# xingchensong/TouchNet

Hardware: AMD Instinct MI355X
Metric: audio+text tokens/sec/node (packed seq, full train step) + step MFU (higher is better)
Workload: dtype bf16

## Files before the change

touchnet_amd/csrc/attn_bwd_fused.hip:

```cpp
#include "attn_common.h"

namespace tn {

namespace fusedkv {

#define TN_FKV_BLOCKS(M)                                                                                              \
  if constexpr (BLK == 0) { M("a0","a1","a2","a3","a4","a5","a6","a7","a8","a9","a10","a11","a12","a13","a14","a15"); } \
  if constexpr (BLK == 1) { M("a16","a17","a18","a19","a20","a21","a22","a23","a24","a25","a26","a27","a28","a29","a30","a31"); } \
  if constexpr (BLK == 2) { M("a32","a33","a34","a35","a36","a37","a38","a39","a40","a41","a42","a43","a44","a45","a46","a47"); } \
  if constexpr (BLK == 3) { M("a48","a49","a50","a51","a52","a53","a54","a55","a56","a57","a58","a59","a60","a61","a62","a63"); } \
  if constexpr (BLK == 4) { M("a64","a65","a66","a67","a68","a69","a70","a71","a72","a73","a74","a75","a76","a77","a78","a79"); } \
  if constexpr (BLK == 5) { M("a80","a81","a82","a83","a84","a85","a86","a87","a88","a89","a90","a91","a92","a93","a94","a95"); } \
  if constexpr (BLK == 6) { M("a96","a97","a98","a99","a100","a101","a102","a103","a104","a105","a106","a107","a108","a109","a110","a111"); } \
  if constexpr (BLK == 7) { M("a112","a113","a114","a115","a116","a117","a118","a119","a120","a121","a122","a123","a124","a125","a126","a127"); }

template <int BLK, bool FIRST>
__device__ __forceinline__ void acc_mfma(bf16x8_t a, bf16x8_t b) {
#define TN_M(...)                                                                                                     \
  if constexpr (FIRST)                                                                                                \
    asm volatile("s_nop 1\n\tv_mfma_f32_32x32x16_bf16 a[%c2:%c3], %0, %1, a[%c2:%c3]" ::"v"(a), "v"(b),             \
                 "n"(16 * BLK), "n"(16 * BLK + 15) : __VA_ARGS__);                                                    \
  else                                                                                                                \
    asm volatile("v_mfma_f32_32x32x16_bf16 a[%c2:%c3], %0, %1, a[%c2:%c3]" ::"v"(a), "v"(b), "n"(16 * BLK),          \
                 "n"(16 * BLK + 15) : __VA_ARGS__)
// ... 21 lines not shown
}

template <int K>
__device__ __forceinline__ void mfma_first(f32x16_t& d, u32x4_t a, bf16x8_t b) {
  asm volatile("s_waitcnt lgkmcnt(%3)\n\tv_mfma_f32_32x32x16_bf16 %0, %1, %2, 0" : "=&v"(d) : "v"(a), "v"(b), "n"(K));
}
template <int K>
__device__ __forceinline__ void mfma_acc(f32x16_t& d, u32x4_t a, bf16x8_t b) {
  asm volatile("s_waitcnt lgkmcnt(%3)\n\tv_mfma_f32_32x32x16_bf16 %0, %1, %2, %0" : "+v"(d) : "v"(a), "v"(b), "n"(K));
}
__device__ __forceinline__ void mfma_result_pad(f32x16_t& d) { asm volatile("s_nop 7\n\ts_nop 4" : "+v"(d)); }

constexpr int g2_ops(int g, bool mask) { return g < 4 ? 4 : g < 6 ? 3 + (mask ? 1 : 0) : 1 + (mask ? 1 : 0); }
constexpr int g2_wait(int s, bool mask) {
  int y = 0;
  if (s < 4) {
    y = 3 - s;
    for (int g = 0; g < s; ++g) y += g2_ops(g, mask);
  } else {
    y = g2_ops(s - 4, mask) - 1;
    for (int g = s - 3; g < s; ++g) y += g2_ops(g, mask);
  }
  return y;
}
static_assert(g2_wait(0, false) == 3 && g2_wait(3, false) == 12 && g2_wait(4, false) == 15 && g2_wait(7, false) == 10 &&
              g2_wait(5, true) == 15 && g2_wait(6, true) == 15 && g2_wait(7, true) == 13, "LDS wait table");

struct QStage {
  int qsb, meta, base, srow;
};

}

template <int D>
__global__ __launch_bounds__(256, 1) void attn_bwd_kv_fused_kernel(
    const bf16_t* __restrict__ Q, const bf16_t* __restrict__ K, const bf16_t* __restrict__ V,
    const bf16_t* __restrict__ dO, const float* __restrict__ LSE2, const float* __restrict__ Delta,
    bf16_t* __restrict__ dK, bf16_t* __restrict__ dV, const int* __restrict__ doc, AttnMeta meta, QView qv, int T,
    int Nh, int Nkv, float scale, float scale_log2, const bf16_t* __restrict__ rcos, const bf16_t* __restrict__ rsin) {
  using namespace fusedkv;
  static_assert(D == 128, "the fused dK/dV pass is built for head_dim 128");
  constexpr int BNK = 128, BQ = 32, NST = 4, SPT = kTile / BQ;
  constexpr int KSTEPS = D / 16, DBLK = D / 32;
  using Tile = PTile<BQ, D>;
  constexpr int IMGB = Tile::SIZE * 2;
  constexpr int NPC = Tile::NP * (BQ / 16);
  constexpr int PPW = NPC / 4;
  constexpr int IPS = 2 * PPW + 1;
  constexpr int STAGEB = 2 * IMGB + 4 * 256;
  constexpr int LCAP = 256;
  using KTile = PTile<32, D>;
  constexpr int KIMGB = KTile::SIZE * 2;
  static_assert(4 * 2 * KIMGB <= NST * STAGEB && 4 * 2 * WholeRows<D>::BYTES <= NST * STAGEB, "private images live in the ring area");
  __shared__ __attribute__((aligned(1024))) char smem[NST * STAGEB + (LCAP + NST + 1) * 16 + 16 + kListPre * 16];
  i32x4_t* slist = reinterpret_cast<i32x4_t*>(smem + NST * STAGEB);
  int* wcount = reinterpret_cast<int*>(smem + NST * STAGEB + (LCAP + NST + 1) * 16);
  i32x4_t* qent = reinterpret_cast<i32x4_t*>(smem + NST * STAGEB + (LCAP + NST + 1) * 16 + 16);

  const int tid = threadIdx.x, lane = tid & 63;
  const int wave = __builtin_amdgcn_readfirstlane(tid >> 6);
  const int l31 = lane & 31, hi = lane >> 5;
  const int kt = blockIdx.y, hk = blockIdx.x, b = blockIdx.z;
  const int G = Nh / Nkv;
  const int k0 = kt * BNK;
  const int wk0 = k0 + 32 * wave;
  const int kvrow = wk0 + l31;
  const bool kvalid = kvrow < T;

  const bool plain = qv.nseg == 1 && qv.off[0] == 0 && qv.row0[0] == 0 && qv.rows[0] == T && qv.rpb == T;
  i32x4_t ql_head = {kListPre + 1, 0, 0, 0}, ql_mine = {0, 0, 0, 0};
  if (plain) {
    const i32x4_t* ql = reinterpret_cast<const i32x4_t*>(meta.qlist) + ((size_t)b * meta.nq128 + kt) * (1 + kListPre);
    ql_head = ql[0];
    if (tid < kListPre) ql_mine = ql[1 + tid];
  }
  i32x4_t ws4[4];
#pragma unroll
  for (int w = 0; w < 4; ++w) {
    ws4[w] = i32x4_t{0x7fffffff, 0, 1, 0};
    if (k0 + 32 * w < T) ws4[w] = reinterpret_cast<const i32x4_t*>(meta.qstat)[(size_t)b * meta.nq32 + (k0 + 32 * w) / 32];
  }
  const int dkdoc = kvalid ? doc[(size_t)b * T + kvrow] : 0;
  {
    const size_t krow_elems = (size_t)Nkv * D;
    const uint32_t k_bytes = (uint32_t)min((size_t)T * krow_elems * 2, (size_t)0x7fffffff);
    const __amdgpu_buffer_rsrc_t rk =
        __builtin_amdgcn_make_buffer_rsrc((void*)(K + (size_t)b * T * krow_elems), 0, k_bytes, 0x00020000);
    const __amdgpu_buffer_rsrc_t rv =
        __builtin_amdgcn_make_buffer_rsrc((void*)(V + (size_t)b * T * krow_elems), 0, k_bytes, 0x00020000);
    const int rrk = lane >> 2;
    const uint32_t voffk = (uint32_t)(((size_t)rrk * krow_elems + 8 * ((lane & 3) ^ ((rrk >> 2) & 3))) * 2);
    char* kpriv = smem + wave * (2 * KIMGB);
#pragma unroll
    for (int pc = 0; pc < KTile::NP * 2; ++pc) {
      const int panel = pc % KTile::NP, rh = pc / KTile::NP;
      const uint32_t vo = (wk0 + 16 * rh + rrk < T) ? voffk : 0x80000000u;
      const uint32_t so = (uint32_t)((((size_t)wk0 + 16 * rh) * krow_elems + (size_t)hk * D + 32 * panel) * 2);
      char* dst = kpriv + panel * (KTile::PSTRIDE * 2) + rh * 1024;
      __builtin_amdgcn_raw_ptr_buffer_load_lds(rk, (lds_ptr_t)dst, 16, vo, so, 0, 0);
      __builtin_amdgcn_raw_ptr_buffer_load_lds(rv, (lds_ptr_t)(dst + KIMGB), 16, vo, so, 0, 0);
    }
  }
  wait_vmcnt<0>();
  asm volatile("" ::"v"(dkdoc));
  bf16x8_t kreg[KSTEPS], vreg[KSTEPS];
  {
    const PRowReader<32, D> krd(l31, hi);
    const bf16_t* ki = reinterpret_cast<const bf16_t*>(smem + wave * (2 * KIMGB));
#pragma unroll
    for (int s2 = 0; s2 < KSTEPS; ++s2) {
      kreg[s2] = krd.operand(ki, 0, s2);
      vreg[s2] = krd.operand(ki + KTile::SIZE, 0, s2);
    }
#pragma unroll
    for (int s2 = 0; s2 < KSTEPS; ++s2) asm volatile("s_waitcnt lgkmcnt(0)" : "+v"(kreg[s2]), "+v"(vreg[s2]));
  }
  const int n_pre = __builtin_amdgcn_readfirstlane(ql_head.x);
  const bool pre = n_pre <= kListPre;
  if (pre && tid < n_pre) qent[tid] = ql_mine;
  __syncthreads();

  const int* m_min = meta.tmin + (size_t)b * meta.nt;
  const int* m_max = meta.tmax + (size_t)b * meta.nt;
  const int* m_minpos = meta.tminpos + (size_t)b * meta.nt;
  const int qt_lo = k0 / kTile;
  const int t0 = 2 * kt, t1 = min(2 * kt + 1, meta.nt - 1);
  int bminpos = 0, bmax = 0, qt_end = 0;
  if (!pre) {
    bminpos = min(m_minpos[t0], m_minpos[t1]);
    bmax = max(m_max[t0], m_max[t1]);
    const int qhi64 = max(meta.kv_hi[(size_t)b * meta.nt + t0], meta.kv_hi[(size_t)b * meta.nt + t1]);
    qt_end = min(qhi64 + 1, meta.nt);
  }
  const int4 wsc = scalarize(ws4[0]);
  const int4 wsc1 = scalarize(ws4[1]), wsc2 = scalarize(ws4[2]), wsc3 = scalarize(ws4[3]);
  const int4 wsw[4] = {wsc, wsc1, wsc2, wsc3};
  int seg_lo[2], seg_n[2];
// ... 84 lines not shown
  auto issue = [&](const QStage& d, int sbase) {
    char* st = smem + sbase;
    const int left = d.meta & 0xff;
#pragma unroll
    for (int i = 0; i < PPW; ++i) {
      const int pc = wave + 4 * i, panel = pc % Tile::NP, rh = pc / Tile::NP;
      const uint32_t vo = (16 * rh + rr < left) ? voff : OOB;
      const uint32_t so = (uint32_t)d.base + (uint32_t)((16 * rh * qrow_elems + 32 * panel) * 2);
      char* dst = st + panel * (Tile::PSTRIDE * 2) + rh * 1024;
      __builtin_amdgcn_raw_ptr_buffer_load_lds(rq, (lds_ptr_t)dst, 16, vo, so, 0, 0);
      __builtin_amdgcn_raw_ptr_buffer_load_lds(rdo, (lds_ptr_t)(dst + IMGB), 16, vo, so, 0, 0);
    }
    const uint32_t va = lane < left ? (uint32_t)lane * 4 : OOB;
    __builtin_amdgcn_raw_ptr_buffer_load_lds(raux, (lds_ptr_t)(st + 2 * IMGB + 256 * wave), 4, va,
                                             wave < 2 ? (uint32_t)d.srow : (uint32_t)d.qsb * 4, 0, 0);
  };

  static_for<2 * DBLK>([&](auto I) { acc_zero<decltype(I)::value>(); });

  const PRowReader<BQ, D> rrd(l31, hi);
  const PTrReader<BQ, D> trd(lane);
  const uint32_t lds0 = (uint32_t)(size_t)(lds_ptr_t)smem;
  const uint32_t trb0 = lds0 + 2 * (uint32_t)trd.t[0], trb1 = lds0 + 2 * (uint32_t)trd.t[1];
  const uint32_t rwb0 = lds0 + 2 * (uint32_t)rrd.a[0], rwb1 = lds0 + 2 * (uint32_t)rrd.a[1];
  const uint32_t auxb = lds0 + 16 * (uint32_t)hi;

  bf16x8_t Pc[2];
  float pf[16];
  f32x16_t dPc;
  bool act_c = false;

  auto trip = [&](auto cur_t, auto next_t, auto mask_t, int qsb_n, const QStage& ahead, int sb_c, int sb_n,
                  int sb_a) {
    constexpr bool CUR = decltype(cur_t)::value, NEXT = decltype(next_t)::value, MASK = decltype(mask_t)::value;
    constexpr bool BOTH = CUR && NEXT;
    u32x2_t th[8][2];
    bf16x8_t tf[8];
    f32x4_t de4[4], le4[4];
    i32x4_t qd4[4];
    u32x4_t rq_[8], rdo_[8];
    f32x16_t S, dPn;
    float pn[16], dsf[16];
    bf16x8_t Pn[2], dSc[2];
    const uint32_t ta0 = trb0 + (uint32_t)sb_c, ta1 = trb1 + (uint32_t)sb_c;
    const uint32_t rn0 = rwb0 + (uint32_t)sb_n, rn1 = rwb1 + (uint32_t)sb_n;
    const uint32_t axc = auxb + (uint32_t)sb_c, axn = auxb + (uint32_t)sb_n;
    auto tr_retire = [&]() {
#pragma unroll
      for (int i = 0; i < 8; ++i) {
        const u32x4_t t = {th[i][0].x, th[i][0].y, th[i][1].x, th[i][1].y};
        tf[i] = __builtin_bit_cast(bf16x8_t, t);
      }
    };
    if constexpr (CUR) {
      static_for<8>([&](auto I) {
        constexpr int i = decltype(I)::value, sp = i >> 2, db = i & 3;
        constexpr int off = 2 * (Tile::SIZE + db * Tile::PSTRIDE + 16 * sp * 32);
        th[i][0] = ds_tr16<off>(ta0);
        th[i][1] = ds_tr16<off + 512>(ta1);
      });
      de4[0] = ds_b128<2 * IMGB + 256, f32x4_t>(axc);
      de4[1] = ds_b128<2 * IMGB + 256 + 32, f32x4_t>(axc);
    }
    wait_vmcnt<IPS>();
    __builtin_amdgcn_s_barrier();
    asm volatile("" ::: "memory");
    issue(ahead, sb_a);
    auto ds_elem = [&dPc, &pf, &de4, &dsf](auto R) {
      constexpr int r = decltype(R)::value;
      float v = pf[r] * (dPc[r] - de4[r >> 2][r & 3]);
      asm volatile("" : "+v"(v));
      dsf[r] = v;
    };
    auto p_elem = [&](auto R) {
      constexpr int r = decltype(R)::value;
      float pv = fast_exp2(S[r] * scale_log2 - le4[r >> 2][r & 3]);
      if constexpr (MASK) {
        const int o = 8 * (r >> 2) + 4 * hi + (r & 3);
        pv = ((kvrow <= qsb_n + o) & (qd4[r >> 2][r & 3] == dkdoc) & (dkdoc > 0)) ? pv : 0.f;
      }
      asm volatile("" : "+v"(pv));
      pn[r] = pv;
    };
    auto pack8 = [&](const float (&p)[16], int sp) {
      const u32x4_t t = {pack2bf(p[8 * sp + 0], p[8 * sp + 1]), pack2bf(p[8 * sp + 2], p[8 * sp + 3]),
                         pack2bf(p[8 * sp + 4], p[8 * sp + 5]), pack2bf(p[8 * sp + 6], p[8 * sp + 7])};
      return __builtin_bit_cast(bf16x8_t, t);
    };
    if constexpr (CUR) {
      asm volatile("s_waitcnt lgkmcnt(0)"
                   : "+v"(th[0][0]), "+v"(th[0][1]), "+v"(th[1][0]), "+v"(th[1][1]), "+v"(th[2][0]), "+v"(th[2][1]),
                     "+v"(th[3][0]), "+v"(th[3][1]), "+v"(th[4][0]), "+v"(th[4][1]), "+v"(th[5][0]), "+v"(th[5][1]),
                     "+v"(th[6][0]), "+v"(th[6][1]), "+v"(th[7][0]), "+v"(th[7][1]), "+v"(de4[0]), "+v"(de4[1]));
      tr_retire();
    }
    static_for<8>([&](auto I) {
      constexpr int i = decltype(I)::value, sp = i >> 2, db = i & 3;
      if constexpr (CUR) {
        acc_mfma<db, i == 0>(tf[i], Pc[sp]);
        ds_elem(std::integral_constant<int, i>{});
        if constexpr (i == 2 || i == 3) de4[i] = ds_b128<2 * IMGB + 256 + 32 * i, f32x4_t>(axc);
      }
      if constexpr (NEXT && i >= 4) {
        constexpr int s = i - 4;
        rq_[s] = ds_b128<2 * ((s >> 1) * Tile::PSTRIDE)>((s & 1) ? rn1 : rn0);
      }
      __builtin_amdgcn_sched_barrier(0);
    });
    if constexpr (CUR) dSc[0] = pack8(dsf, 0);
    if constexpr (CUR && !NEXT) asm volatile("s_waitcnt lgkmcnt(0)" : "+v"(de4[2]), "+v"(de4[3]));
    static_for<8>([&](auto I) {
      constexpr int s = decltype(I)::value;
      if constexpr (NEXT) {
        constexpr int k = BOTH ? g2_wait(s, MASK) : 0;
        if constexpr (s == 0 && CUR)
          asm volatile("s_waitcnt lgkmcnt(%2)" : "+v"(de4[2]), "+v"(de4[3]) : "n"(k));
        if constexpr (s == 0) mfma_first<k>(S, rq_[0], kreg[0]);
        else mfma_acc<k>(S, rq_[s], kreg[s]);
        if constexpr (s < 4) rq_[s + 4] = ds_b128<2 * (((s + 4) >> 1) * Tile::PSTRIDE)>((s & 1) ? rn1 : rn0);
      }
      if constexpr (CUR) {
        ds_elem(std::integral_constant<int, 8 + s>{});
        if constexpr (s < 6) {
          constexpr int first = s < 4 ? 3 * s : 12 + 2 * (s - 4), cnt = s < 4 ? 3 : 2;
          static_for<cnt>([&](auto J) {
            constexpr int x = first + decltype(J)::value, i = x >> 1, half = x & 1;
            constexpr int off = 2 * ((i & 3) * Tile::PSTRIDE + 16 * (i >> 2) * 32) + 512 * half;
            th[i][half] = ds_tr16<off>(half ? ta1 : ta0);
          });
        }
      }
      if constexpr (NEXT && s >= 4) {
        le4[s - 4] = ds_b128<2 * IMGB + 32 * (s - 4), f32x4_t>(axn);
        if constexpr (MASK) qd4[s - 4] = ds_b128<2 * IMGB + 512 + 32 * (s - 4), i32x4_t>(axn);
      }
      __builtin_amdgcn_sched_barrier(0);
    });
    if constexpr (CUR) dSc[1] = pack8(dsf, 1);
    if constexpr (CUR && NEXT && MASK) {
      asm volatile("s_waitcnt lgkmcnt(0)"
                   : "+v"(th[0][0]), "+v"(th[0][1]), "+v"(th[1][0]), "+v"(th[1][1]), "+v"(th[2][0]), "+v"(th[2][1]),
                     "+v"(th[3][0]), "+v"(th[3][1]), "+v"(th[4][0]), "+v"(th[4][1]), "+v"(th[5][0]), "+v"(th[5][1]),
                     "+v"(th[6][0]), "+v"(th[6][1]), "+v"(th[7][0]), "+v"(th[7][1]), "+v"(le4[0]), "+v"(le4[1]),
                     "+v"(le4[2]), "+v"(le4[3]), "+v"(qd4[0]), "+v"(qd4[1]), "+v"(qd4[2]), "+v"(qd4[3]));
    } else if constexpr (CUR && NEXT) {
      asm volatile("s_waitcnt lgkmcnt(0)"
                   : "+v"(th[0][0]), "+v"(th[0][1]), "+v"(th[1][0]), "+v"(th[1][1]), "+v"(th[2][0]), "+v"(th[2][1]),
                     "+v"(th[3][0]), "+v"(th[3][1]), "+v"(th[4][0]), "+v"(th[4][1]), "+v"(th[5][0]), "+v"(th[5][1]),
                     "+v"(th[6][0]), "+v"(th[6][1]), "+v"(th[7][0]), "+v"(th[7][1]), "+v"(le4[0]), "+v"(le4[1]),
                     "+v"(le4[2]), "+v"(le4[3]));
    } else if constexpr (CUR) {
      asm volatile("s_waitcnt lgkmcnt(0)"
                   : "+v"(th[0][0]), "+v"(th[0][1]), "+v"(th[1][0]), "+v"(th[1][1]), "+v"(th[2][0]), "+v"(th[2][1]),
                     "+v"(th[3][0]), "+v"(th[3][1]), "+v"(th[4][0]), "+v"(th[4][1]), "+v"(th[5][0]), "+v"(th[5][1]),
                     "+v"(th[6][0]), "+v"(th[6][1]), "+v"(th[7][0]), "+v"(th[7][1]));
    } else if constexpr (NEXT && MASK) {
      asm volatile("s_waitcnt lgkmcnt(0)" : "+v"(le4[0]), "+v"(le4[1]), "+v"(le4[2]), "+v"(le4[3]), "+v"(qd4[0]),
                   "+v"(qd4[1]), "+v"(qd4[2]), "+v"(qd4[3]));
    } else if constexpr (NEXT) {
      asm volatile("s_waitcnt lgkmcnt(0)" : "+v"(le4[0]), "+v"(le4[1]), "+v"(le4[2]), "+v"(le4[3]));
    }
    if constexpr (CUR) tr_retire();
    if constexpr (NEXT && !CUR) mfma_result_pad(S);
    static_for<8>([&](auto I) {
      constexpr int i = decltype(I)::value, sp = i >> 2, db = i & 3;
      if constexpr (CUR) acc_mfma<DBLK + db, i == 0>(tf[i], dSc[sp]);
      if constexpr (NEXT) {
        if constexpr (i == 0 && CUR) asm volatile("s_nop 4" : "+v"(S));
        p_elem(std::integral_constant<int, i>{});
        rdo_[i] = ds_b128<2 * (Tile::SIZE + (i >> 1) * Tile::PSTRIDE)>((i & 1) ? rn1 : rn0);
      }
      __builtin_amdgcn_sched_barrier(0);
    });
    if constexpr (NEXT) {
      Pn[0] = pack8(pn, 0);
      asm volatile("" : "+v"(Pn[0]));
    }
    static_for<8>([&](auto I) {
      constexpr int s = decltype(I)::value;
      if constexpr (NEXT) {
        if constexpr (s == 0) mfma_first<7>(dPn, rdo_[0], vreg[0]);
        else mfma_acc<7 - s>(dPn, rdo_[s], vreg[s]);
        p_elem(std::integral_constant<int, 8 + s>{});
      }
      __builtin_amdgcn_sched_barrier(0);
    });
    if constexpr (NEXT) {
      Pn[1] = pack8(pn, 1);
      asm volatile("" : "+v"(Pn[1]));
// ... 11 lines not shown
    {
      const QStage s0 = entry(0), s1 = entry(1);
      issue(s0, 1 * STAGEB);
      issue(s1, 2 * STAGEB);
    }
    int q1 = __builtin_amdgcn_readfirstlane(slist[0].x), m1 = __builtin_amdgcn_readfirstlane(slist[0].y);
    int q2 = __builtin_amdgcn_readfirstlane(slist[1].x), m2 = __builtin_amdgcn_readfirstlane(slist[1].y);
    act_c = false;
    i32x4_t e0 = slist[2];
    int it = -1, sb_c = 0, sb_n = 0, sb_a = 0;
    bool act_n = false, mask_n = false;
    QStage ahead;
    auto head = [&]() {
      const int4 ea = scalarize(e0);
      ahead = QStage{ea.x, ea.y, ea.z, ea.w};
      e0 = slist[it + 4];
      const int sc = (it + 1) & 3;
      sb_c = sc * STAGEB;
      sb_n = ((sc + 1) & 3) * STAGEB;
      sb_a = ((sc + 3) & 3) * STAGEB;
      act_n = (m1 & act_bit) != 0;
      mask_n = (m1 & mask_bit) != 0;
    };
    auto tail = [&]() {
      act_c = act_n;
      q1 = q2;
      m1 = m2;
      q2 = ahead.qsb;
      m2 = ahead.meta;
      ++it;
    };
    using T_ = std::true_type;
    using F_ = std::false_type;
    head();
    while (true) {
      if (act_c && act_n && !mask_n) {
        do {
          trip(T_{}, T_{}, F_{}, q1, ahead, sb_c, sb_n, sb_a);
          tail();
          if (it >= n) break;
          head();
        } while (act_n && !mask_n);
        if (it >= n) break;
        continue;
      }
      if (act_c) {
        if (act_n) trip(T_{}, T_{}, T_{}, q1, ahead, sb_c, sb_n, sb_a);
        else trip(T_{}, F_{}, F_{}, q1, ahead, sb_c, sb_n, sb_a);
      } else {
        if (act_n) {
          if (mask_n) trip(F_{}, T_{}, T_{}, q1, ahead, sb_c, sb_n, sb_a);
          else trip(F_{}, T_{}, F_{}, q1, ahead, sb_c, sb_n, sb_a);
        } else {
          trip(F_{}, F_{}, F_{}, q1, ahead, sb_c, sb_n, sb_a);
        }
      }
      tail();
      if (it >= n) break;
      head();
    }
    wait_vmcnt<0>();
    __syncthreads();
  }

  asm volatile("s_nop 15\n\ts_nop 15");
  {
    using WR = WholeRows<D>;
    constexpr int CPR = WR::CPR, RPI = WR::RPI, NI = WR::NI;
    const int cc = lane % CPR, r0 = lane / CPR;
    const bool rot = rcos != nullptr;
    u32x4_t c4[NI] = {}, s4[NI] = {};
    if (rot) {
#pragma unroll
      for (int i = 0; i < NI; ++i) {
        const size_t to = ((size_t)b * T + min(wk0 + i * RPI + r0, T - 1)) * (D / 2) + (cc & (CPR / 2 - 1)) * 8;
        c4[i] = *reinterpret_cast<const u32x4_t*>(rcos + to);
        s4[i] = *reinterpret_cast<const u32x4_t*>(rsin + to);
      }
    }
    char* obv = smem + wave * (2 * WR::BYTES);
    char* obk = obv + WR::BYTES;
    static_for<DBLK>([&](auto DB) {
      constexpr int db = decltype(DB)::value;
      static_for<4>([&](auto R4) {
        constexpr int r4 = decltype(R4)::value;
        u32x2_t o;
        o.x = pack2bf(acc_read<16 * db + 4 * r4 + 0>(), acc_read<16 * db + 4 * r4 + 1>());
        o.y = pack2bf(acc_read<16 * db + 4 * r4 + 2>(), acc_read<16 * db + 4 * r4 + 3>());
        *WR::put(obv, l31, hi, db, r4) = o;
        o.x = pack2bf(acc_read<64 + 16 * db + 4 * r4 + 0>() * scale, acc_read<64 + 16 * db + 4 * r4 + 1>() * scale);
        o.y = pack2bf(acc_read<64 + 16 * db + 4 * r4 + 2>() * scale, acc_read<64 + 16 * db + 4 * r4 + 3>() * scale);
        *WR::put(obk, l31, hi, db, r4) = o;
      });
    });
    const size_t off = (((size_t)b * T + wk0) * Nkv + hk) * D + cc * 8;
#pragma unroll
    for (int i = 0; i < NI; ++i) {
      const int row = i * RPI + r0;
      const u32x4_t v4 = *WR::get(obv, row, cc);
      u32x4_t k4 = *WR::get(obk, row, cc);
      if (rot) {
        const u32x4_t p4 = *WR::get(obk, row, cc ^ (CPR / 2));
        k4 = rope_grad_chunk(k4, p4, c4[i], s4[i], cc >= CPR / 2);
      }
      if (wk0 + row < T) {
        *reinterpret_cast<u32x4_t*>(dV + off + (size_t)row * Nkv * D) = v4;
        *reinterpret_cast<u32x4_t*>(dK + off + (size_t)row * Nkv * D) = k4;
      }
    }
  }
}

void launch_attn_bwd_kv_fused128(const bf16_t* Q, const bf16_t* K, const bf16_t* V, const bf16_t* dO,
                                 const float* lse2, const float* delta, bf16_t* dK, bf16_t* dV, const int* doc,
                                 AttnMeta m, QView qv, int B, int T, int Nh, int Nkv, float scale, float sl2,
                                 const bf16_t* rcos, const bf16_t* rsin, hipStream_t st) {
  dim3 gk(Nkv, (T + 127) / 128, B), block(256);
  hipLaunchKernelGGL((attn_bwd_kv_fused_kernel<128>), gk, block, 0, st, Q, K, V, dO, lse2, delta, dK, dV, doc, m, qv,
                     T, Nh, Nkv, scale, sl2, rcos, rsin);
}

}
```

touchnet_amd/csrc/attn_common.h:

```cpp
#pragma once
#include <type_traits>
#include <utility>

#include "common.h"

namespace tn {

typedef __attribute__((ext_vector_type(4))) uint32_t u32x4_t;
typedef __attribute__((ext_vector_type(4))) int i32x4_t;
typedef __attribute__((ext_vector_type(4))) float f32x4_t;
typedef __attribute__((ext_vector_type(2))) uint32_t u32x2_t;
typedef __attribute__((ext_vector_type(2))) float f32x2_t;
typedef __attribute__((address_space(3))) void* lds_ptr_t;

__device__ __forceinline__ f32x16_t mfma32(bf16x8_t a, bf16x8_t b, f32x16_t c) {
  return __builtin_amdgcn_mfma_f32_32x32x16_bf16(a, b, c, 0, 0, 0);
}
__device__ __forceinline__ float max3(float a, float b, float c) { return fmaxf(fmaxf(a, b), c); }
__device__ __forceinline__ bf16x8_t as_bf16x8(uint4 v) {
  u32x4_t t = {v.x, v.y, v.z, v.w};
  return __builtin_bit_cast(bf16x8_t, t);
}
__device__ __forceinline__ bf16x8_t as_bf16x8(uint2 lo, uint2 hi) {
  u32x4_t t = {lo.x, lo.y, hi.x, hi.y};
// ... 10 lines not shown
  u32x2_t r;
  asm volatile("ds_read_b64_tr_b16 %0, %1 offset:%2" : "=v"(r) : "v"(addr), "n"(OFF));
  return r;
}
template <int OFF, class V = u32x4_t>
__device__ __forceinline__ V ds_b128(uint32_t addr) {
  V r;
  asm volatile("ds_read_b128 %0, %1 offset:%2" : "=v"(r) : "v"(addr), "n"(OFF));
  return r;
}
template <class F, int... I>
__device__ __forceinline__ void static_for_impl(F& f, std::integer_sequence<int, I...>) {
  (f(std::integral_constant<int, I>{}), ...);
}
template <int N, class F>
__device__ __forceinline__ void static_for(F&& f) {
  static_for_impl(f, std::make_integer_sequence<int, N>{});
}

constexpr int kTile = 64;

constexpr int kListPre = 64;
struct AttnMeta {
  const int* tmin;
  const int* tmax;
  const int* tminpos;
  const int* q_lo;
  const int* kv_hi;
  int nt;
  const int* qstat;
  const int* klist;
  int nq32, nq128;
  const int* qlist;
};
__host__ inline int attn_meta_ints(int B, int T) {
  const int nt = (T + kTile - 1) / kTile, nq32 = (T + 31) / 32, nq128 = (T + 127) / 128;
  return 5 * B * nt + 4 * B * nq32 + 2 * (4 + 4 * kListPre) * B * nq128;
}
__host__ inline AttnMeta make_attn_meta(const int* meta, int B, int T) {
  const int nt = (T + kTile - 1) / kTile, n = B * nt, nq32 = (T + 31) / 32, nq128 = (T + 127) / 128;
  return AttnMeta{meta, meta + n, meta + 2 * n, meta + 3 * n, meta + 4 * n, nt,
                  meta + 5 * n, meta + 5 * n + 4 * B * nq32, nq32, nq128,
                  meta + 5 * n + 4 * B * nq32 + (4 + 4 * kListPre) * B * nq128};
}

struct QView {
  int nseg;
  int row0[2], rows[2], off[2];
  int rpb;
  int kv_tpc;
  unsigned long long kv_mask;
  int bidir;
  __host__ static QView whole(int T) { return QView{1, {0, 0}, {T, 0}, {0, 0}, T, 0, ~0ull, 0}; }
  __device__ __forceinline__ bool kv_tile_on(int j) const { return kv_tpc == 0 || ((kv_mask >> (j / kv_tpc)) & 1ull); }
  __host__ __device__ int tiles(int s, int bm) const { return s < nseg ? (rows[s] + bm - 1) / bm : 0; }
  __device__ __forceinline__ void tile(int idx, int bm, int& l0, int& g0, int& left) const {
    const int n0 = tiles(0, bm);
    const int s = idx >= n0 ? 1 : 0;
    const int lt = idx - (s ? n0 : 0);
    l0 = row0[s] + lt * bm;
    g0 = off[s] + lt * bm;
    left = rows[s] - lt * bm;
  }
};

__host__ inline bool attn_shape_ok(int B, int T, int Nh, int Nkv, int D) {
  return B > 0 && T > 0 && Nh > 0 && Nkv > 0 && Nh % Nkv == 0 && (D == 64 || D == 128);
}

__host__ inline int seg_view(int nseg, const int* segs, int rows_per_batch, int T, QView* out) {
  if (nseg < 1 || nseg > 2 || segs == nullptr || rows_per_batch <= 0 || T <= 0) return TN_EINVAL;
  QView qv = {nseg, {0, 0}, {0, 0}, {0, 0}, rows_per_batch, 0, ~0ull, 0};
  for (int s = 0; s < nseg; ++s) {
    const int row0 = segs[3 * s], rows = segs[3 * s + 1], off = segs[3 * s + 2];
    if (rows <= 0 || off < 0 || row0 < 0) return TN_EINVAL;
    if ((long long)off + rows > T || (long long)row0 + rows > rows_per_batch) return TN_EINVAL;
// ... 166 lines not shown
```

touchnet_amd/csrc/attn_fwd.hip:

```cpp
#include "attn_common.h"

namespace tn {

__global__ void attn_meta_stats_kernel(const int* __restrict__ doc, int* tmin, int* tmax, int* tminpos, int B, int T,
                                       int nt) {
  const int idx = blockIdx.x * blockDim.x + threadIdx.x;
  if (idx >= B * nt) return;
  const int b = idx / nt, t = idx % nt;
  int mn = 0x7fffffff, mx = 0, mnp = 0x7fffffff;
  for (int i = 0; i < kTile; ++i) {
    const int p = t * kTile + i;
    const int d = p < T ? doc[(size_t)b * T + p] : 0;
    mn = min(mn, d);
    mx = max(mx, d);
    if (d > 0) mnp = min(mnp, d);
  }
  tmin[idx] = mn;
  tmax[idx] = mx;
  tminpos[idx] = mnp;
}

__global__ void attn_meta_range_kernel(const int* __restrict__ tmax, const int* __restrict__ tminpos, int* q_lo,
                                       int* kv_hi, int B, int nt) {
  const int idx = blockIdx.x * blockDim.x + threadIdx.x;
// ... 51 lines not shown
  for (int base = j_lo; base <= t1; base += 64) {
    const int j = base + lane;
    const bool ok = j <= t1 && tile_may_interact(bminpos, bmax, mp[j <= t1 ? j : t1], mx[j <= t1 ? j : t1]);
    const unsigned long long bal = __ballot(ok);
    const int pos = count + __popcll(bal & ((1ull << lane) - 1ull));
    if (ok && pos < kListPre) out[1 + pos] = make_int4(j, mn[j], mx[j], mp[j]);
    count += __popcll(bal);
  }
  if (lane == 0) out[0] = make_int4(count, qt, 0, 0);
}

__global__ void attn_meta_qlist_kernel(const int* __restrict__ tmin, const int* __restrict__ tmax,
                                       const int* __restrict__ tminpos, const int* __restrict__ kv_hi,
                                       int* __restrict__ qlist, int B, int nt, int nq128) {
  const int kt = blockIdx.x, b = blockIdx.y, lane = threadIdx.x;
  const int* mn = tmin + (size_t)b * nt;
  const int* mx = tmax + (size_t)b * nt;
  const int* mp = tminpos + (size_t)b * nt;
  const int t0 = 2 * kt, t1 = min(2 * kt + 1, nt - 1);
  const int bminpos = min(mp[t0], mp[t1]), bmax = max(mx[t0], mx[t1]);
  const int qt_end = min(max(kv_hi[(size_t)b * nt + t0], kv_hi[(size_t)b * nt + t1]) + 1, nt);
  int4* out = reinterpret_cast<int4*>(qlist + ((size_t)b * nq128 + kt) * (4 + 4 * kListPre));
  int count = 0;
  for (int base = t0; base < qt_end; base += 64) {
    const int t = base + lane;
    const int tc = t < qt_end ? t : t0;
    const bool ok = t < qt_end && tile_may_interact(mp[tc], mx[tc], bminpos, bmax);
    const unsigned long long bal = __ballot(ok);
    const int pos = count + __popcll(bal & ((1ull << lane) - 1ull));
    if (ok && pos < kListPre) out[1 + pos] = make_int4(t, mn[t], mx[t], mp[t]);
    count += __popcll(bal);
  }
  if (lane == 0) out[0] = make_int4(count, kt, 0, 0);
}

__global__ void attn_merge_kernel(const bf16_t* __restrict__ oa, const float* __restrict__ la,
                                  const bf16_t* __restrict__ ob, const float* __restrict__ lb, bf16_t* __restrict__ o,
                                  float* __restrict__ l, int B, int R, int Nh, int D) {
  const int dv = D / 8;
  const size_t idx = (size_t)blockIdx.x * blockDim.x + threadIdx.x;
  const size_t total = (size_t)B * R * Nh * dv;
  if (idx >= total) return;
  const int d8 = (int)(idx % dv);
  const int h = (int)((idx / dv) % Nh);
  const size_t br = idx / ((size_t)dv * Nh);
  const int b = (int)(br / R), r = (int)(br % R);
  const size_t li = ((size_t)b * Nh + h) * R + r;
  const float a = la[li], c = lb[li];
  const bool ea = a == INFINITY, ec = c == INFINITY;
  const float m = ea ? c : (ec ? a : fmaxf(a, c));
  const float wa = ea ? 0.f : fast_exp2(a - m), wc = ec ? 0.f : fast_exp2(c - m);
  const float tot = wa + wc;
  const float inv = tot > 0.f ? 1.f / tot : 0.f;
  Vec16<bf16_t> va, vc, vo;
  va.load(oa + idx * 8);
  vc.load(ob + idx * 8);
  float fa[8], fc[8], fo[8];
  va.unpack(fa);
  vc.unpack(fc);
#pragma unroll
  for (int e = 0; e < 8; ++e) fo[e] = (wa * fa[e] + wc * fc[e]) * inv;
  vo.pack(fo);
  vo.store(o + idx * 8);
  if (d8 == 0) l[li] = tot > 0.f ? m + log2f(tot) : INFINITY;
}

}

using namespace tn;

int tn_attn_fwd_pp_launch(const void* q, const void* k, const void* v, void* o, float* lse2, const int* doc,
                          AttnMeta m, QView qv, int B, int T, int Nh, int Nkv, int D, float sl2, hipStream_t st);
int tn_attn_fwd_stream_launch(const void* q, const void* k, const void* v, void* o, float* lse2, const int* doc,
                              AttnMeta m, QView qv, int B, int T, int Nh, int Nkv, int D, float sl2, hipStream_t st);

static bool fwd_pingpong(int T, int D, int nt, const QView& qv) {
  return T >= 32768 && D == 128 && !qv.bidir && nt <= 1024;
}

extern "C" {

int tn_attn_meta_ints(int B, int T) { return attn_meta_ints(B, T); }

int tn_attn_build_meta(const int* doc, int* meta, int B, int T, void* stream) {
  if (B <= 0 || T <= 0) return TN_EINVAL;
  const int nt = (T + kTile - 1) / kTile, n = B * nt;
  hipStream_t st = (hipStream_t)stream;
  hipLaunchKernelGGL(attn_meta_stats_kernel, dim3((n + 127) / 128), dim3(128), 0, st, doc, meta, meta + n,
                     meta + 2 * n, B, T, nt);
  TN_LAUNCH_CHECK();
  hipLaunchKernelGGL(attn_meta_range_kernel, dim3((n + 127) / 128), dim3(128), 0, st, meta + n, meta + 2 * n,
                     meta + 3 * n, meta + 4 * n, B, nt);
  TN_LAUNCH_CHECK();
  const AttnMeta m = make_attn_meta(meta, B, T);
  hipLaunchKernelGGL(attn_meta_qstat_kernel, dim3((B * m.nq32 + 127) / 128), dim3(128), 0, st, doc,
                     const_cast<int*>(m.qstat), B, T, m.nq32);
  TN_LAUNCH_CHECK();
  hipLaunchKernelGGL(attn_meta_klist_kernel, dim3(m.nq128, B), dim3(64), 0, st, m.tmin, m.tmax, m.tminpos, m.q_lo,
                     const_cast<int*>(m.klist), B, nt, m.nq128);
  TN_LAUNCH_CHECK();
  hipLaunchKernelGGL(attn_meta_qlist_kernel, dim3(m.nq128, B), dim3(64), 0, st, m.tmin, m.tmax, m.tminpos, m.kv_hi,
                     const_cast<int*>(m.qlist), B, nt, m.nq128);
  TN_LAUNCH_CHECK();
  return TN_OK;
}

static int attn_fwd_launch(const void* q, const void* k, const void* v, void* o, float* lse2, const int* doc,
                           const int* meta, int B, int T, int Nh, int Nkv, int D, float scale, QView qv,
                           void* stream) {
  if (!attn_shape_ok(B, T, Nh, Nkv, D)) return TN_EINVAL;
  const int nt = (T + kTile - 1) / kTile;
  const AttnMeta m = make_attn_meta(meta, B, T);
  const float sl2 = scale * kLog2e;
  hipStream_t st = (hipStream_t)stream;
  if (fwd_pingpong(T, D, nt, qv)) return tn_attn_fwd_pp_launch(q, k, v, o, lse2, doc, m, qv, B, T, Nh, Nkv, D, sl2, st);
  return tn_attn_fwd_stream_launch(q, k, v, o, lse2, doc, m, qv, B, T, Nh, Nkv, D, sl2, st);
}

int tn_attn_fwd(const void* q, const void* k, const void* v, void* o, float* lse2, const int* doc, const int* meta,
                int B, int T, int Nh, int Nkv, int D, float scale, void* stream) {
  const QView qv = QView::whole(T);
  return attn_fwd_launch(q, k, v, o, lse2, doc, meta, B, T, Nh, Nkv, D, scale, qv, stream);
}

int tn_attn_fwd_bidir(const void* q, const void* k, const void* v, void* o, float* lse2, const int* doc,
                      const int* meta, int B, int T, int Nh, int Nkv, int D, float scale, void* stream) {
  QView qv = QView::whole(T);
  qv.bidir = 1;
  return attn_fwd_launch(q, k, v, o, lse2, doc, meta, B, T, Nh, Nkv, D, scale, qv, stream);
}

int tn_attn_fwd_seg(const void* q, const void* k, const void* v, void* o, float* lse2, const int* doc,
                    const int* meta, int B, int T, int Nh, int Nkv, int D, float scale, int nseg, const int* segs,
                    int rows_per_batch, void* stream) {
  QView qv;
// ... 27 lines not shown
```

touchnet_amd/library.py:

```python
from __future__ import annotations

import ctypes
from typing import List, Optional, Tuple

import torch
from torch import Tensor
from torch.library import custom_op

from . import _C

NS = "mi355_touch"
_p, _cur = _C.ptr, _C.stream


def _lib():
    return _C.lib()


def _c(t: Tensor) -> Tensor:
    return t if t.is_contiguous() else t.contiguous()


def _empty0(like: Tensor) -> Tensor:
    return like.new_empty(0)
# ... 335 lines not shown
                  scale: float, cos: Tensor, sin: Tensor, stacked: bool) -> Tensor:
    B, T, Nh, D = q.shape
    if not (cos.dtype == torch.bfloat16 and sin.dtype == torch.bfloat16 and cos.is_contiguous() and sin.is_contiguous()
            and cos.numel() == B * T * (D // 2) and sin.numel() == cos.numel()):
        raise _C.KernelError("attn_bwd_rope: cos / sin are the bf16 [B * T, head_dim / 2] tables of rope_tables")
    return _attn_backward("tn_attn_bwd_rope", "stacked" if stacked else "flat", q, k, v, o, do, lse2, doc, meta, scale,
                          (_p(cos), _p(sin)))


@custom_op(f"{NS}::attn_bwd_seg", mutates_args=(), device_types="cuda")
def attn_bwd_seg(q: Tensor, k: Tensor, v: Tensor, o: Tensor, do: Tensor, lse2: Tensor, doc: Tensor, meta: Tensor,
                 scale: float, segs: List[int], rows_per_batch: int) -> Tuple[Tensor, Tensor, Tensor]:
    return _attn_backward("tn_attn_bwd_seg", "tuple", q, k, v, o, do, lse2, doc, meta, scale,
                          _segs_tail(segs, q.shape[1]))


for _op, _layout in ((attn_bwd, "tuple"), (attn_bwd_bidir, "tuple"), (attn_bwd_stacked, "stacked"), (attn_bwd_seg, "tuple")):
    _op.register_fake(lambda q, k, *rest, _layout=_layout: attn_grads(q, k, _layout)[0])
attn_bwd_rope.register_fake(lambda q, k, *rest: attn_grads(q, k, "stacked" if rest[-1] else "flat")[0])


def _attn_causal_grads(q, k, *rest):
    if q.shape == k.shape:
        return attn_bwd_stacked(q, k, *rest).unbind(0)
    return attn_bwd(q, k, *rest)


_attn_autograd(attn_fwd, _attn_causal_grads)
_attn_autograd(attn_fwd_bidir, attn_bwd_bidir)
_attn_autograd(attn_fwd_seg, attn_bwd_seg)


def attn_meta_ints(B: int, T: int) -> int:
    nt, nq32, nq128 = (T + 63) // 64, (T + 31) // 32, (T + 127) // 128
    return B * (5 * nt + 4 * nq32 + 2 * (4 + 4 * 64) * nq128)


@custom_op(f"{NS}::attn_build_meta", mutates_args=(), device_types="cuda")
def attn_build_meta(doc: Tensor) -> Tensor:
    B, T = doc.shape
    meta = torch.empty(_lib().tn_attn_meta_ints(B, T), dtype=torch.int32, device=doc.device)
    _C.check(_lib().tn_attn_build_meta(_p(doc), _p(meta), B, T, _cur()), "tn_attn_build_meta")
    return meta


@attn_build_meta.register_fake
def _(doc):
    return doc.new_empty(attn_meta_ints(*doc.shape), dtype=torch.int32)


@custom_op(f"{NS}::attn_merge", mutates_args=(), device_types="cuda")
def attn_merge(o_a: Tensor, lse2_a: Tensor, o_b: Tensor, lse2_b: Tensor) -> Tuple[Tensor, Tensor]:
    o_a, o_b, la, lb = _c(o_a), _c(o_b), _c(lse2_a), _c(lse2_b)
    B, R, Nh, D = o_a.shape
    o, lse2 = torch.empty_like(o_a), torch.empty_like(la)
    _C.check(_lib().tn_attn_merge(_p(o_a), _p(la), _p(o_b), _p(lb), _p(o), _p(lse2), B, R, Nh, D, _cur()),
             "tn_attn_merge")
    return o, lse2


@attn_merge.register_fake
def _(o_a, lse2_a, o_b, lse2_b):
    return (torch.empty_like(o_a, memory_format=torch.contiguous_format),
            torch.empty_like(lse2_a, memory_format=torch.contiguous_format))


@custom_op(f"{NS}::ce_fwd", mutates_args=(), device_types="cuda")
def ce_fwd(logits: Tensor, labels: Tensor, sentence_lens: Tensor, num_sentence: Tensor,
# ... 835 lines not shown
```

Baseline: 23940.

## Use per-row doc-end bounds for cheaper masking in fused dK/dV backward

Adds per-token doc_end/doc_start and a per-batch contiguity flag to attention metadata, built by new meta kernels. For batches whose documents are contiguous runs, the fused dK/dV kernel runs a variant that masks with one unsigned range compare against the row's doc end. That avoids loading per-query doc ids from LDS and the three-way compare. Non-contiguous batches still use the original doc-id mask. Two kernel launches now run (each exits early for batches it does not handle), and metadata build gains three extra launches.

```diff
diff --git a/touchnet_amd/csrc/attn_bwd_fused.hip b/touchnet_amd/csrc/attn_bwd_fused.hip
--- a/touchnet_amd/csrc/attn_bwd_fused.hip
+++ b/touchnet_amd/csrc/attn_bwd_fused.hip
@@ -77,7 +77,7 @@
 
 }
 
-template <int D>
+template <int D, int PRED>
 __global__ __launch_bounds__(256, 1) void attn_bwd_kv_fused_kernel(
     const bf16_t* __restrict__ Q, const bf16_t* __restrict__ K, const bf16_t* __restrict__ V,
     const bf16_t* __restrict__ dO, const float* __restrict__ LSE2, const float* __restrict__ Delta,
@@ -113,6 +113,7 @@
   const bool kvalid = kvrow < T;
 
   const bool plain = qv.nseg == 1 && qv.off[0] == 0 && qv.row0[0] == 0 && qv.rows[0] == T && qv.rpb == T;
+  if (plain ? (meta.contig[b] != 0) != (PRED == 2) : PRED == 2) return;
   i32x4_t ql_head = {kListPre + 1, 0, 0, 0}, ql_mine = {0, 0, 0, 0};
   if (plain) {
     const i32x4_t* ql = reinterpret_cast<const i32x4_t*>(meta.qlist) + ((size_t)b * meta.nq128 + kt) * (1 + kListPre);
@@ -126,6 +127,10 @@
     if (k0 + 32 * w < T) ws4[w] = reinterpret_cast<const i32x4_t*>(meta.qstat)[(size_t)b * meta.nq32 + (k0 + 32 * w) / 32];
   }
   const int dkdoc = kvalid ? doc[(size_t)b * T + kvrow] : 0;
+  int dkend = kvrow - 1;
+  if constexpr (PRED == 2) {
+    if (kvalid) dkend = meta.doc_end[(size_t)b * T + kvrow];
+  }
   {
     const size_t krow_elems = (size_t)Nkv * D;
     const uint32_t k_bytes = (uint32_t)min((size_t)T * krow_elems * 2, (size_t)0x7fffffff);
@@ -148,6 +153,9 @@
   }
   wait_vmcnt<0>();
   asm volatile("" ::"v"(dkdoc));
+  if constexpr (PRED == 2) asm volatile("" ::"v"(dkend));
+  const uint32_t klen = (uint32_t)(dkend - kvrow + 1);
+  const int kq0 = kvrow - 4 * hi;
   bf16x8_t kreg[KSTEPS], vreg[KSTEPS];
   {
     const PRowReader<32, D> krd(l31, hi);
@@ -298,8 +306,11 @@
 
   auto trip = [&](auto cur_t, auto next_t, auto mask_t, int qsb_n, const QStage& ahead, int sb_c, int sb_n,
                   int sb_a) {
-    constexpr bool CUR = decltype(cur_t)::value, NEXT = decltype(next_t)::value, MASK = decltype(mask_t)::value;
+    constexpr bool CUR = decltype(cur_t)::value, NEXT = decltype(next_t)::value;
+    constexpr int MASK = decltype(mask_t)::value;
+    constexpr bool QD = MASK == 1;
     constexpr bool BOTH = CUR && NEXT;
+    const int qk = qsb_n - kq0;
     u32x2_t th[8][2];
     bf16x8_t tf[8];
     f32x4_t de4[4], le4[4];
@@ -341,10 +352,11 @@
     auto p_elem = [&](auto R) {
       constexpr int r = decltype(R)::value;
       float pv = fast_exp2(S[r] * scale_log2 - le4[r >> 2][r & 3]);
-      if constexpr (MASK) {
+      if constexpr (MASK == 1) {
         const int o = 8 * (r >> 2) + 4 * hi + (r & 3);
         pv = ((kvrow <= qsb_n + o) & (qd4[r >> 2][r & 3] == dkdoc) & (dkdoc > 0)) ? pv : 0.f;
       }
+      if constexpr (MASK == 2) pv = (uint32_t)(qk + (8 * (r >> 2) + (r & 3))) < klen ? pv : 0.f;
       asm volatile("" : "+v"(pv));
       pn[r] = pv;
     };
@@ -378,7 +390,7 @@
     static_for<8>([&](auto I) {
       constexpr int s = decltype(I)::value;
       if constexpr (NEXT) {
-        constexpr int k = BOTH ? g2_wait(s, MASK) : 0;
+        constexpr int k = BOTH ? g2_wait(s, QD) : 0;
         if constexpr (s == 0 && CUR)
           asm volatile("s_waitcnt lgkmcnt(%2)" : "+v"(de4[2]), "+v"(de4[3]) : "n"(k));
         if constexpr (s == 0) mfma_first<k>(S, rq_[0], kreg[0]);
@@ -398,12 +410,12 @@
       }
       if constexpr (NEXT && s >= 4) {
         le4[s - 4] = ds_b128<2 * IMGB + 32 * (s - 4), f32x4_t>(axn);
-        if constexpr (MASK) qd4[s - 4] = ds_b128<2 * IMGB + 512 + 32 * (s - 4), i32x4_t>(axn);
+        if constexpr (QD) qd4[s - 4] = ds_b128<2 * IMGB + 512 + 32 * (s - 4), i32x4_t>(axn);
       }
       __builtin_amdgcn_sched_barrier(0);
     });
     if constexpr (CUR) dSc[1] = pack8(dsf, 1);
-    if constexpr (CUR && NEXT && MASK) {
+    if constexpr (CUR && NEXT && QD) {
       asm volatile("s_waitcnt lgkmcnt(0)"
                    : "+v"(th[0][0]), "+v"(th[0][1]), "+v"(th[1][0]), "+v"(th[1][1]), "+v"(th[2][0]), "+v"(th[2][1]),
                      "+v"(th[3][0]), "+v"(th[3][1]), "+v"(th[4][0]), "+v"(th[4][1]), "+v"(th[5][0]), "+v"(th[5][1]),
@@ -420,7 +432,7 @@
                    : "+v"(th[0][0]), "+v"(th[0][1]), "+v"(th[1][0]), "+v"(th[1][1]), "+v"(th[2][0]), "+v"(th[2][1]),
                      "+v"(th[3][0]), "+v"(th[3][1]), "+v"(th[4][0]), "+v"(th[4][1]), "+v"(th[5][0]), "+v"(th[5][1]),
                      "+v"(th[6][0]), "+v"(th[6][1]), "+v"(th[7][0]), "+v"(th[7][1]));
-    } else if constexpr (NEXT && MASK) {
+    } else if constexpr (NEXT && QD) {
       asm volatile("s_waitcnt lgkmcnt(0)" : "+v"(le4[0]), "+v"(le4[1]), "+v"(le4[2]), "+v"(le4[3]), "+v"(qd4[0]),
                    "+v"(qd4[1]), "+v"(qd4[2]), "+v"(qd4[3]));
     } else if constexpr (NEXT) {
@@ -498,11 +510,13 @@
     };
     using T_ = std::true_type;
     using F_ = std::false_type;
+    using M0 = std::integral_constant<int, 0>;
+    using MK = std::integral_constant<int, PRED>;
     head();
     while (true) {
       if (act_c && act_n && !mask_n) {
         do {
-          trip(T_{}, T_{}, F_{}, q1, ahead, sb_c, sb_n, sb_a);
+          trip(T_{}, T_{}, M0{}, q1, ahead, sb_c, sb_n, sb_a);
           tail();
           if (it >= n) break;
           head();
@@ -511,14 +525,14 @@
         continue;
       }
       if (act_c) {
-        if (act_n) trip(T_{}, T_{}, T_{}, q1, ahead, sb_c, sb_n, sb_a);
-        else trip(T_{}, F_{}, F_{}, q1, ahead, sb_c, sb_n, sb_a);
+        if (act_n) trip(T_{}, T_{}, MK{}, q1, ahead, sb_c, sb_n, sb_a);
+        else trip(T_{}, F_{}, M0{}, q1, ahead, sb_c, sb_n, sb_a);
       } else {
         if (act_n) {
-          if (mask_n) trip(F_{}, T_{}, T_{}, q1, ahead, sb_c, sb_n, sb_a);
-          else trip(F_{}, T_{}, F_{}, q1, ahead, sb_c, sb_n, sb_a);
+          if (mask_n) trip(F_{}, T_{}, MK{}, q1, ahead, sb_c, sb_n, sb_a);
+          else trip(F_{}, T_{}, M0{}, q1, ahead, sb_c, sb_n, sb_a);
         } else {
-          trip(F_{}, F_{}, F_{}, q1, ahead, sb_c, sb_n, sb_a);
+          trip(F_{}, F_{}, M0{}, q1, ahead, sb_c, sb_n, sb_a);
         }
       }
       tail();
@@ -582,7 +596,10 @@
                                  AttnMeta m, QView qv, int B, int T, int Nh, int Nkv, float scale, float sl2,
                                  const bf16_t* rcos, const bf16_t* rsin, hipStream_t st) {
   dim3 gk(Nkv, (T + 127) / 128, B), block(256);
-  hipLaunchKernelGGL((attn_bwd_kv_fused_kernel<128>), gk, block, 0, st, Q, K, V, dO, lse2, delta, dK, dV, doc, m, qv,
+  if (qv.nseg == 1 && qv.off[0] == 0 && qv.row0[0] == 0 && qv.rows[0] == T && qv.rpb == T)
+    hipLaunchKernelGGL((attn_bwd_kv_fused_kernel<128, 2>), gk, block, 0, st, Q, K, V, dO, lse2, delta, dK, dV, doc, m, qv,
+                       T, Nh, Nkv, scale, sl2, rcos, rsin);
+  hipLaunchKernelGGL((attn_bwd_kv_fused_kernel<128, 1>), gk, block, 0, st, Q, K, V, dO, lse2, delta, dK, dV, doc, m, qv,
                      T, Nh, Nkv, scale, sl2, rcos, rsin);
 }
 
diff --git a/touchnet_amd/csrc/attn_common.h b/touchnet_amd/csrc/attn_common.h
--- a/touchnet_amd/csrc/attn_common.h
+++ b/touchnet_amd/csrc/attn_common.h
@@ -66,16 +66,25 @@
   const int* klist;
   int nq32, nq128;
   const int* qlist;
-};
+  const int* doc_end;
+  const int* doc_start;
+  const int* contig;
+};
+__host__ __device__ constexpr int attn_meta_pad4(int n) { return (n + 3) & ~3; }
+__host__ inline int attn_meta_tile_ints(int B, int T) {
+  const int nt = (T + kTile - 1) / kTile, nq32 = (T + 31) / 32, nq128 = (T + 127) / 128;
+  return attn_meta_pad4(5 * B * nt + 4 * B * nq32 + 2 * (4 + 4 * kListPre) * B * nq128);
+}
 __host__ inline int attn_meta_ints(int B, int T) {
-  const int nt = (T + kTile - 1) / kTile, nq32 = (T + 31) / 32, nq128 = (T + 127) / 128;
-  return 5 * B * nt + 4 * B * nq32 + 2 * (4 + 4 * kListPre) * B * nq128;
+  return attn_meta_tile_ints(B, T) + 2 * attn_meta_pad4(B * T) + attn_meta_pad4(B);
 }
 __host__ inline AttnMeta make_attn_meta(const int* meta, int B, int T) {
   const int nt = (T + kTile - 1) / kTile, n = B * nt, nq32 = (T + 31) / 32, nq128 = (T + 127) / 128;
+  const int* pos = meta + attn_meta_tile_ints(B, T);
   return AttnMeta{meta, meta + n, meta + 2 * n, meta + 3 * n, meta + 4 * n, nt,
                   meta + 5 * n, meta + 5 * n + 4 * B * nq32, nq32, nq128,
-                  meta + 5 * n + 4 * B * nq32 + (4 + 4 * kListPre) * B * nq128};
+                  meta + 5 * n + 4 * B * nq32 + (4 + 4 * kListPre) * B * nq128,
+                  pos, pos + attn_meta_pad4(B * T), pos + 2 * attn_meta_pad4(B * T)};
 }
 
 struct QView {
diff --git a/touchnet_amd/csrc/attn_fwd.hip b/touchnet_amd/csrc/attn_fwd.hip
--- a/touchnet_amd/csrc/attn_fwd.hip
+++ b/touchnet_amd/csrc/attn_fwd.hip
@@ -107,6 +107,53 @@
     count += __popcll(bal);
   }
   if (lane == 0) out[0] = make_int4(count, kt, 0, 0);
+}
+
+__global__ void attn_meta_runs_init_kernel(int* __restrict__ runs, int* __restrict__ contig, int B, int T) {
+  const int idx = blockIdx.x * blockDim.x + threadIdx.x;
+  if (idx < B * T) runs[idx] = 0;
+  if (idx < B) contig[idx] = 1;
+}
+__global__ void attn_meta_runs_kernel(const int* __restrict__ doc, int* __restrict__ runs, int* __restrict__ contig, int B,
+                                      int T) {
+  const int idx = blockIdx.x * blockDim.x + threadIdx.x;
+  if (idx >= B * T) return;
+  const int b = idx / T, t = idx % T;
+  const int d = doc[idx];
+  if (d <= 0 || (t > 0 && doc[idx - 1] == d)) return;
+  if (d > T || atomicAdd(&runs[(size_t)b * T + d - 1], 1) > 0) contig[b] = 0;
+}
+__global__ void attn_meta_bounds_kernel(const int* __restrict__ doc, const int* __restrict__ tmin,
+                                        const int* __restrict__ tmax, int* __restrict__ doc_end,
+                                        int* __restrict__ doc_start, int B, int T, int nt) {
+  const int idx = blockIdx.x * blockDim.x + threadIdx.x;
+  if (idx >= B * T) return;
+  const int b = idx / T, t = idx % T;
+  const int* row = doc + (size_t)b * T;
+  const int* mn = tmin + (size_t)b * nt;
+  const int* mx = tmax + (size_t)b * nt;
+  const int d = row[t];
+  int e = t - 1, s = t + 1;
+  if (d > 0) {
+    e = t;
+    while ((e + 1) % kTile != 0 && e + 1 < T && row[e + 1] == d) ++e;
+    if ((e + 1) % kTile == 0) {
+      int j = (e + 1) / kTile;
+      while (j < nt && mn[j] == d && mx[j] == d) ++j;
+      e = j * kTile - 1;
+      while (e + 1 < T && row[e + 1] == d) ++e;
+    }
+    s = t;
+    while (s % kTile != 0 && row[s - 1] == d) --s;
+    if (s % kTile == 0) {
+      int j = s / kTile - 1;
+      while (j >= 0 && mn[j] == d && mx[j] == d) --j;
+      s = (j + 1) * kTile;
+      while (s > 0 && row[s - 1] == d) --s;
+    }
+  }
+  doc_end[idx] = e;
+  doc_start[idx] = s;
 }
 
 __global__ void attn_merge_kernel(const bf16_t* __restrict__ oa, const float* __restrict__ la,
@@ -158,7 +205,7 @@
 int tn_attn_meta_ints(int B, int T) { return attn_meta_ints(B, T); }
 
 int tn_attn_build_meta(const int* doc, int* meta, int B, int T, void* stream) {
-  if (B <= 0 || T <= 0) return TN_EINVAL;
+  if (B <= 0 || T <= 0 || (long long)B * T > 0x3fffffff) return TN_EINVAL;
   const int nt = (T + kTile - 1) / kTile, n = B * nt;
   hipStream_t st = (hipStream_t)stream;
   hipLaunchKernelGGL(attn_meta_stats_kernel, dim3((n + 127) / 128), dim3(128), 0, st, doc, meta, meta + n,
@@ -176,6 +223,15 @@
   TN_LAUNCH_CHECK();
   hipLaunchKernelGGL(attn_meta_qlist_kernel, dim3(m.nq128, B), dim3(64), 0, st, m.tmin, m.tmax, m.tminpos, m.kv_hi,
                      const_cast<int*>(m.qlist), B, nt, m.nq128);
+  TN_LAUNCH_CHECK();
+  const dim3 gp((B * T + 255) / 256), bp(256);
+  int* runs = const_cast<int*>(m.doc_start);
+  hipLaunchKernelGGL(attn_meta_runs_init_kernel, gp, bp, 0, st, runs, const_cast<int*>(m.contig), B, T);
+  TN_LAUNCH_CHECK();
+  hipLaunchKernelGGL(attn_meta_runs_kernel, gp, bp, 0, st, doc, runs, const_cast<int*>(m.contig), B, T);
+  TN_LAUNCH_CHECK();
+  hipLaunchKernelGGL(attn_meta_bounds_kernel, gp, bp, 0, st, doc, m.tmin, m.tmax, const_cast<int*>(m.doc_end),
+                     const_cast<int*>(m.doc_start), B, T, nt);
   TN_LAUNCH_CHECK();
   return TN_OK;
 }
diff --git a/touchnet_amd/library.py b/touchnet_amd/library.py
--- a/touchnet_amd/library.py
+++ b/touchnet_amd/library.py
@@ -391,8 +391,40 @@
 
 
 def attn_meta_ints(B: int, T: int) -> int:
+    return sum(n for _, n in attn_meta_sections(B, T).values())
+
+
+def attn_meta_sections(B: int, T: int) -> dict:
     nt, nq32, nq128 = (T + 63) // 64, (T + 31) // 32, (T + 127) // 128
-    return B * (5 * nt + 4 * nq32 + 2 * (4 + 4 * 64) * nq128)
+    pad4 = lambda n: (n + 3) & ~3
+    rec = (4 + 4 * 64) * B * nq128
+    tiles = 5 * B * nt + 4 * B * nq32 + 2 * rec
+    sizes = [(name, B * nt) for name in ("tmin", "tmax", "tminpos", "q_lo", "kv_hi")]
+    sizes += [("qstat", 4 * B * nq32), ("klist", rec), ("qlist", rec + pad4(tiles) - tiles)]
+    sizes += [("doc_end", pad4(B * T)), ("doc_start", pad4(B * T)), ("contig", pad4(B))]
+    out, off = {}, 0
+    for name, n in sizes:
+        out[name] = (off, n)
+        off += n
+    return out
+
+
+def attn_doc_bounds(doc: Tensor) -> Tuple[Tensor, Tensor, Tensor]:
+    B, T = doc.shape
+    d = doc.long()
+    pos = torch.arange(T, device=doc.device).expand(B, T)
+    first = torch.ones_like(d, dtype=torch.bool)
+    first[:, 1:] = d[:, 1:] != d[:, :-1]
+    last = torch.ones_like(first)
+    last[:, :-1] = first[:, 1:]
+    start = torch.where(first, pos, torch.zeros_like(pos)).cummax(1).values
+    end = torch.where(last, pos, torch.full_like(pos, T)).flip(1).cummin(1).values.flip(1)
+    pad = d <= 0
+    start, end = torch.where(pad, pos + 1, start), torch.where(pad, pos - 1, end)
+    runs = torch.zeros(B, T + 1, dtype=torch.long, device=doc.device)
+    runs.scatter_add_(1, d.clamp(0, T), (first & ~pad & (d <= T)).long())
+    contig = (runs.amax(1) <= 1) & ~((d > T).any(1))
+    return end.int(), start.int(), contig.int()
 
 
 @custom_op(f"{NS}::attn_build_meta", mutates_args=(), device_types="cuda")
```

After: 23920. About the same (-0.1%).
